# Kang-ChangWoo/audio-depth-estimation

Hardware: AMD Instinct MI355X
Metric: depth-maps/sec (train step) (higher is better)
Workload: dtype bf16; 1 GPU; unetbaseline_model unet_256 (ngf 64) train step, BatVisionV2-shaped 256x256, batch 32/GPU, Combined L1+SIlog loss, clip 1.0, AdamW; global_batch=32, image_size=256, launch=hipGraph, parallelism=dp1

## Files before the change

audio-depth-estimation_amd/csrc/epilogue.h:

```cpp
#pragma once
#include "adn_common.h"

__device__ __forceinline__ float adn_final_act(float y, int kind) {
  return kind == 1 ? 1.0f / (1.0f + __expf(-y)) : (kind == 2 ? y : fmaxf(y, 0.0f));
}

template <typename T>
__device__ __forceinline__ void epi_scalar(int epi, const AdnEpiSeg& sg, int64_t op, int nl, float v,
                                           float& s1, float& s2) {
  const int64_t idx = op * sg.channels + nl;
  if (epi == ADN_EPI_RAW) {
    reinterpret_cast<float*>(sg.out0)[idx] = v;
  } else if (epi == ADN_EPI_Z_STATS) {
    if (sg.bias) v += sg.bias[nl];
    ElemTraits<T>::store(reinterpret_cast<T*>(sg.out0) + idx, v);
    s1 += v;
    s2 += v * v;
  } else if (epi == ADN_EPI_ACT) {
    float y = v;
    if (sg.scale) y = y * sg.scale[nl];
    if (sg.shift) y += sg.shift[nl];
    if (sg.bias) y += sg.bias[nl];
    if (sg.out0) ElemTraits<T>::store(reinterpret_cast<T*>(sg.out0) + idx, y > 0.f ? y : y * sg.slope);
    if (sg.out1) ElemTraits<T>::store(reinterpret_cast<T*>(sg.out1) + idx, fmaxf(y, 0.f));
// ... 31 lines not shown
    u32x4_t c0 = p[0], c1 = p[1];
    Chunk<float>::unpack(c0, f);
    Chunk<float>::unpack(c1, f + 4);
  }
}
template <typename T>
__device__ __forceinline__ void store8(void* base, int64_t idx, const float* f) {
  if constexpr (sizeof(T) == 2) {
    *reinterpret_cast<u32x4_t*>(reinterpret_cast<uint16_t*>(base) + idx) = Chunk<uint16_t>::pack(f);
  } else {
    u32x4_t* p = reinterpret_cast<u32x4_t*>(reinterpret_cast<float*>(base) + idx);
    p[0] = Chunk<float>::pack(f);
    p[1] = Chunk<float>::pack(f + 4);
  }
}

struct EpiCols {
  float a[8], b[8];
};

template <typename T>
__device__ __forceinline__ void epi_cols_init(int epi, const AdnEpiSeg& sg, int nl, EpiCols& c) {
#pragma unroll
  for (int e = 0; e < 8; ++e) {
    c.a[e] = 1.0f;
    c.b[e] = 0.0f;
  }
  if (epi == ADN_EPI_ACT) {
#pragma unroll
    for (int e = 0; e < 8; ++e) {
      if (sg.scale) c.a[e] = sg.scale[nl + e];
      if (sg.shift) c.b[e] = sg.shift[nl + e];
      if (sg.bias) c.b[e] += sg.bias[nl + e];
    }
  } else if (epi == ADN_EPI_BWD && sg.partials) {
#pragma unroll
    for (int e = 0; e < 8; ++e) {
      c.a[e] = sg.mean[nl + e];
      c.b[e] = sg.istd[nl + e];
    }
  } else if ((epi == ADN_EPI_FINAL || epi == ADN_EPI_Z_STATS) && sg.bias) {
#pragma unroll
    for (int e = 0; e < 8; ++e) c.b[e] = sg.bias[nl + e];
  } else if (epi == ADN_EPI_ADD) {
#pragma unroll
    for (int e = 0; e < 8; ++e) {
      if (sg.scale) c.a[e] = sg.final_act ? sg.scale[0] : sg.scale[nl + e];
      if (sg.bias) c.b[e] = sg.bias[nl + e];
    }
  }
}

template <typename T>
__device__ __forceinline__ void epi_vec8(int epi, const AdnEpiSeg& sg, const EpiCols& c, int64_t op, int nl,
                                         const float* v, float* s1, float* s2) {
  const int64_t idx = op * sg.channels + nl;
  if (epi == ADN_EPI_RAW) {
    store8<float>(sg.out0, idx, v);
  } else if (epi == ADN_EPI_Z_STATS) {
    float zb[8];
#pragma unroll
    for (int e = 0; e < 8; ++e) zb[e] = v[e] + c.b[e];
    store8<T>(sg.out0, idx, zb);
#pragma unroll
    for (int e = 0; e < 8; ++e) {
      s1[e] += zb[e];
      s2[e] += zb[e] * zb[e];
    }
  } else if (epi == ADN_EPI_ACT) {
    float y[8], o[8];
#pragma unroll
    for (int e = 0; e < 8; ++e) y[e] = v[e] * c.a[e] + c.b[e];
    if (sg.out0) {
#pragma unroll
      for (int e = 0; e < 8; ++e) o[e] = y[e] > 0.f ? y[e] : y[e] * sg.slope;
      store8<T>(sg.out0, idx, o);
    }
    if (sg.out1) {
#pragma unroll
      for (int e = 0; e < 8; ++e) o[e] = fmaxf(y[e], 0.f);
      store8<T>(sg.out1, idx, o);
    }
  } else if (epi == ADN_EPI_BWD) {
    float r[8], g[8];
    load8<T>(sg.ref, idx, r);
#pragma unroll
    for (int e = 0; e < 8; ++e) g[e] = v[e] * (r[e] > 0.f ? 1.0f : sg.slope);
    if (sg.accumulate) {
      float old[8];
      load8<T>(sg.out0, idx, old);
#pragma unroll
      for (int e = 0; e < 8; ++e) g[e] += old[e];
    }
    store8<T>(sg.out0, idx, g);
    if (sg.partials) {
      float z[8];
      load8<T>(sg.z, idx, z);
#pragma unroll
      for (int e = 0; e < 8; ++e) {
        s1[e] += g[e];
        s2[e] += g[e] * ((z[e] - c.a[e]) * c.b[e]);
      }
    }
  } else if (epi == ADN_EPI_ADD) {
    float g[8];
#pragma unroll
    for (int e = 0; e < 8; ++e) g[e] = (v[e] + c.b[e]) * c.a[e];
    if (sg.ref) {
      float r[8];
      load8<T>(sg.ref, idx, r);
#pragma unroll
      for (int e = 0; e < 8; ++e) g[e] += r[e];
    }
    if (sg.accumulate) {
      float old[8];
      load8<T>(sg.out0, idx, old);
#pragma unroll
      for (int e = 0; e < 8; ++e) g[e] += old[e];
    }
    store8<T>(sg.out0, idx, g);
  } else {
    float o[8];
#pragma unroll
    for (int e = 0; e < 8; ++e) o[e] = adn_final_act(v[e] + c.b[e], sg.final_act);
    store8<float>(sg.out0, idx, o);
  }
}

__device__ __forceinline__ void epi_bwd_pre8(const AdnEpiSeg& sg, const EpiCols& c, int64_t op, int nl, const float* v,
                                             const u32x4_t& ref_raw, const u32x4_t& old_raw, const u32x4_t& z_raw,
                                             float* s1, float* s2) {
  const int64_t idx = op * sg.channels + nl;
  float r[8], g[8];
  Chunk<uint16_t>::unpack(ref_raw, r);
#pragma unroll
  for (int e = 0; e < 8; ++e) g[e] = v[e] * (r[e] > 0.f ? 1.0f : sg.slope);
  if (sg.accumulate) {
    float old[8];
    Chunk<uint16_t>::unpack(old_raw, old);
#pragma unroll
    for (int e = 0; e < 8; ++e) g[e] += old[e];
  }
  store8<uint16_t>(sg.out0, idx, g);
  if (sg.partials) {
    float z[8];
    Chunk<uint16_t>::unpack(z_raw, z);
#pragma unroll
    for (int e = 0; e < 8; ++e) {
      s1[e] += g[e];
      s2[e] += g[e] * ((z[e] - c.a[e]) * c.b[e]);
    }
  }
}
```

audio-depth-estimation_amd/csrc/igemm.hip:

```cpp
#include <stdarg.h>
#include <stdio.h>
#include <stdlib.h>

#include <mutex>

#include "epilogue.h"

namespace {

struct Tune {
  int bm = 0, bn = 0, ns = 0, noa = 0, nob = 0, skip = 0, patch = 1, tall = 1, pair = 1, tinycap = 4, bn_t2 = 0, onepx = 1, ring = 1, ring_sched = 1, ring_epi = 0, ring_geom = -1, ring_hs = 0, ring64n = 1;
};
const Tune& tune() {
  static Tune t;
  static std::once_flag once;
  std::call_once(once, [] {
    if (const char* e = getenv("ADN_IGEMM_BM")) t.bm = atoi(e);
    if (const char* e = getenv("ADN_IGEMM_BN")) t.bn = atoi(e);
    if (const char* e = getenv("ADN_IGEMM_NS")) t.ns = atoi(e);
#ifdef ADN_TIMING_KNOBS
    if (const char* e = getenv("ADN_IGEMM_NOA")) t.noa = atoi(e);
    if (const char* e = getenv("ADN_IGEMM_NOB")) t.nob = atoi(e);
    if (const char* e = getenv("ADN_IGEMM_SKIP")) t.skip = atoi(e);
#endif
    if (const char* e = getenv("ADN_IGEMM_PATCH")) t.patch = atoi(e);
    if (const char* e = getenv("ADN_IGEMM_TALL")) t.tall = atoi(e);
    if (const char* e = getenv("ADN_IGEMM_PAIR")) t.pair = atoi(e);
    if (const char* e = getenv("ADN_IGEMM_TINYCAP")) t.tinycap = atoi(e);
    if (const char* e = getenv("ADN_IGEMM_ONEPX")) t.onepx = atoi(e);
    if (const char* e = getenv("ADN_IGEMM_BN_T2")) t.bn_t2 = atoi(e);
    if (const char* e = getenv("ADN_IGEMM_RING")) t.ring = atoi(e);
    if (const char* e = getenv("ADN_IGEMM_RING_SCHED")) t.ring_sched = atoi(e);
    if (const char* e = getenv("ADN_IGEMM_RING_EPI")) t.ring_epi = atoi(e);
    if (const char* e = getenv("ADN_IGEMM_RING_GEOM")) t.ring_geom = atoi(e);
    if (const char* e = getenv("ADN_IGEMM_RING_HS")) t.ring_hs = atoi(e);
    if (const char* e = getenv("ADN_IGEMM_RING_N64")) t.ring64n = atoi(e);
  });
  return t;
}

struct KParams {
  const void* in0;
  const void* in1;
  const void* w;
  int Hs, Ws, C0, C1, N;
  int ks;
  int wstride;
  int Msmall;
  int ksteps;
  int nsplit;
  int tiles_m, tiles_n;
  int epi;
  AdnEpiSeg seg[2];
  float* slab;
  unsigned rec_a, rec_b;
  int skip;
  int onepx;
  int lgW, lgH;
};


__device__ __forceinline__ int xcd_remap(int bid, int nwg) {
  const int q = nwg >> 3, r = nwg & 7, xcd = bid & 7;
  return (xcd < r ? xcd * (q + 1) : r * (q + 1) + (xcd - r) * q) + (bid >> 3);
}

template <int N>
__device__ __forceinline__ void wait_vmcnt() {
  asm volatile("s_waitcnt vmcnt(%0) lgkmcnt(0)" ::"n"(N) : "memory");
}

template <int BM, int BN, int NWN, int NTHR>
struct TileEpi {
  static constexpr int NW = NTHR / 64;
  static constexpr int WN = BN / NWN;
  static constexpr int NT = WN / 16, MT = 4;
  static constexpr int CPR = BN / 8;
  static constexpr int RSTEP = NTHR / CPR;
  static constexpr int RPT = BM / RSTEP;
  static constexpr int LDC = BN + 4;
  static constexpr int lds_bytes = BM * LDC * 4;
};
enum class EpiPre { None, All, NoOld };
template <int RPT, EpiPre PRE>
struct EpiPreRegs {
  u32x4_t r[PRE == EpiPre::None ? 1 : RPT], o[PRE == EpiPre::All ? RPT : 1], z[PRE == EpiPre::None ? 1 : RPT];
};

template <int BM, int BN, int NWN, int NTHR, EpiPre PRE, typename RowOp>
__device__ __forceinline__ void tile_epi_prefetch(const KParams& p, int tile_n, RowOp row_op,
                                                  EpiPreRegs<TileEpi<BM, BN, NWN, NTHR>::RPT, PRE>& pre) {
  using E = TileEpi<BM, BN, NWN, NTHR>;
  if constexpr (PRE != EpiPre::None) {
    const int tid = threadIdx.x;
    const int n0 = tile_n * BN + (tid % E::CPR) * 8, rsub = tid / E::CPR;
    const bool first = n0 < p.seg[0].channels;
    const AdnEpiSeg& sq = first ? p.seg[0] : p.seg[1];
    const int nl0 = first ? n0 : n0 - p.seg[0].channels;
#pragma unroll
    for (int k = 0; k < E::RPT; ++k) {
      pre.r[k] = pre.z[k] = u32x4_t{0u, 0u, 0u, 0u};
      if constexpr (PRE == EpiPre::All) pre.o[k] = u32x4_t{0u, 0u, 0u, 0u};
      int64_t op;
      if (row_op(rsub + E::RSTEP * k, op)) {
        const int64_t idx = op * sq.channels + nl0;
        pre.r[k] = *reinterpret_cast<const u32x4_t*>(reinterpret_cast<const uint16_t*>(sq.ref) + idx);
        if constexpr (PRE == EpiPre::All) {
          if (sq.accumulate) pre.o[k] = *reinterpret_cast<const u32x4_t*>(reinterpret_cast<const uint16_t*>(sq.out0) + idx);
        }
        if (sq.partials) pre.z[k] = *reinterpret_cast<const u32x4_t*>(reinterpret_cast<const uint16_t*>(sq.z) + idx);
      }
    }
  }
}

template <typename T, int BM, int BN, int NWN, int NTHR, EpiPre PRE, typename RowOp>
__device__ __forceinline__ void tile_epi_finish(char* smem, const KParams& p, const f32x4_t (&acc)[4][BN / NWN / 16], int tile_n,
                                                int64_t prow, RowOp row_op, float* slab, bool pre_on,
                                                const EpiPreRegs<TileEpi<BM, BN, NWN, NTHR>::RPT, PRE>& pre) {
  using E = TileEpi<BM, BN, NWN, NTHR>;
  const int tid = threadIdx.x, lane = tid & 63;
  const int wave = __builtin_amdgcn_readfirstlane(tid >> 6);
  const int wm = wave / NWN, wn = wave % NWN;
  const int frow = lane & 15, fq = lane >> 4;
  __syncthreads();
  float* ct = reinterpret_cast<float*>(smem);
#pragma unroll
  for (int i = 0; i < E::MT; ++i)
#pragma unroll
    for (int j = 0; j < E::NT; ++j)
#pragma unroll
      for (int r = 0; r < 4; ++r)
        ct[(wm * 64 + i * 16 + 4 * fq + r) * E::LDC + wn * E::WN + j * 16 + frow] = acc[i][j][r];
  __syncthreads();

  const int cg = tid % E::CPR, rsub = tid / E::CPR;
  const int n0 = tile_n * BN + cg * 8;
  int epi = p.epi;
  AdnEpiSeg sg;
  int nl;
  if (slab != nullptr) {
    epi = ADN_EPI_RAW;
    sg = p.seg[0];
    sg.out0 = slab;
    sg.channels = p.N;
    sg.partials = nullptr;
    nl = n0;
  } else if (n0 < p.seg[0].channels) {
    sg = p.seg[0];
    nl = n0;
  } else {
    sg = p.seg[1];
    nl = n0 - p.seg[0].channels;
  }
  EpiCols cols;
  epi_cols_init<T>(epi, sg, nl, cols);
  float s1[8], s2[8];
#pragma unroll
  for (int e = 0; e < 8; ++e) s1[e] = s2[e] = 0.f;

#pragma unroll
  for (int k = 0; k < E::RPT; ++k) {
    const int row = rsub + E::RSTEP * k;
    int64_t op;
    if (!row_op(row, op)) continue;
    float v[8];
    const f32x4_t v0 = *reinterpret_cast<const f32x4_t*>(ct + row * E::LDC + cg * 8);
    const f32x4_t v1 = *reinterpret_cast<const f32x4_t*>(ct + row * E::LDC + cg * 8 + 4);
#pragma unroll
    for (int e = 0; e < 4; ++e) {
      v[e] = v0[e];
      v[4 + e] = v1[e];
    }
    if constexpr (PRE != EpiPre::None) {
      if (pre_on) {
        if constexpr (PRE == EpiPre::NoOld) {
          u32x4_t old = {0u, 0u, 0u, 0u};
          if (sg.accumulate) old = *reinterpret_cast<const u32x4_t*>(reinterpret_cast<const uint16_t*>(sg.out0) + op * sg.channels + nl);
          epi_bwd_pre8(sg, cols, op, nl, v, pre.r[k], old, pre.z[k], s1, s2);
        } else {
          epi_bwd_pre8(sg, cols, op, nl, v, pre.r[k], pre.o[k], pre.z[k], s1, s2);
        }
        continue;
      }
    }
    epi_vec8<T>(epi, sg, cols, op, nl, v, s1, s2);
  }

  if ((p.seg[0].partials != nullptr || p.seg[1].partials != nullptr) && (epi == ADN_EPI_Z_STATS || epi == ADN_EPI_BWD)) {
// ... 428 lines not shown
    const int soff = (t0 * Cin + (c << 5)) * 2;
    char* dst = Bl + (s & 1) * BBUF + wave * 1024;
#pragma unroll
    for (int k = 0; k < BK_; ++k) __builtin_amdgcn_raw_ptr_buffer_load_lds(rsw, (lptr_t)(dst + k * 4096), 16, bvo[k], soff, 0, 0);
  };

  f32x4_t acc[MT][NT];
#pragma unroll
  for (int i = 0; i < MT; ++i)
#pragma unroll
    for (int j = 0; j < NT; ++j) acc[i][j] = f32x4_t{0.f, 0.f, 0.f, 0.f};

  auto row_op = [&](int row, int64_t& op) -> bool {
    const int oy = oy0 + (row >> 4);
    const int ox = PAIR ? (row & 7) : ox0 + (row & 15);
    const int ib = PAIR ? tb + ((row >> 3) & 1) : tb;
    if constexpr (S2 || S1) op = ((int64_t)ib * Hs + oy) * Ws + ox;
    else op = ((int64_t)ib * Hl + 2 * oy + ph) * Wl + 2 * ox + pw;
    return true;
  };
  constexpr EpiPre EPRE = !PRE ? EpiPre::None : ((S2 || S1) ? EpiPre::NoOld : EpiPre::All);
  const bool pre_on = PRE && p.epi == ADN_EPI_BWD;
  EpiPreRegs<Cfg::Epi::RPT, EPRE> pre;
  if (pre_on) tile_epi_prefetch<BM, BN, NWN, NTHR, EPRE>(p, tile_n, row_op, pre);

#pragma unroll
  for (int ss = 0; ss < SEG_STEPS; ++ss) issue_patch(0, ss);
  issue_b(0);

  const int frow = lane & 15, fq = lane >> 4;
  const int qb0 = wm * 4 * MW + frow + (PAIR ? (frow >> 3) : 0);

  int s = 0;
  for (int sg = 0; sg < nseg; ++sg) {
    const char* Pb = Pl + (sg & 1) * PBUF;
#pragma unroll
    for (int ss = 0; ss < SEG_STEPS; ++ss, ++s) {
      wait_vmcnt<0>();
      __builtin_amdgcn_s_barrier();
      asm volatile("" ::: "memory");
      if (s + 1 < nsteps) issue_b(s + 1);
      if (sg + 1 < nseg) issue_patch(sg + 1, ss);
      const char* Bb = Bl + (s & 1) * BBUF;
#pragma unroll
      for (int e = 0; e < TPS; ++e) {
        int qoff;
        if constexpr (S2) qoff = ((e * (TH + 1)) + (ss >> 1)) * MW + (ss & 1);
        else if constexpr (S1) qoff = ss * MW + e;
        else qoff = (adn_t2_dy(ph, ss) - ymin) * MW + (adn_t2_dy(pw, e) - xmin);
        u32x4_t af[MT], bf[NT];
#pragma unroll
        for (int i = 0; i < MT; ++i) {
          const int q = qb0 + i * MW + qoff;
          af[i] = *reinterpret_cast<const u32x4_t*>(Pb + q * 64 + ((fq ^ (((q >> 2) & 1) << 1)) << 4));
        }
#pragma unroll
        for (int j = 0; j < NT; ++j) {
          const int row = wn * WN + j * 16 + frow;
          bf[j] = *reinterpret_cast<const u32x4_t*>(Bb + e * (BN * 64) + row * 64 + ((fq ^ (((row >> 2) & 1) << 1)) << 4));
        }
#pragma unroll
        for (int i = 0; i < MT; ++i)
#pragma unroll
          for (int j = 0; j < NT; ++j) mma_tile<T>(af[i], bf[j], acc[i][j]);
      }
    }
  }
  tile_epi_finish<T, BM, BN, NWN, NTHR, EPRE>(smem, p, acc, tile_n, (int64_t)phase * p.tiles_m + tile_m, row_op, nullptr, pre_on, pre);
#endif
}

#include "igemm_ring.h"

template <typename T, int GEOM>
__global__ __launch_bounds__(256) void igemm_direct_kernel(KParams p) {
  const int Hs = p.Hs, Ws = p.Ws, Hl = 2 * Hs, Wl = 2 * Ws;
  const int Cin = p.C0 + p.C1;
  const int64_t mout = (GEOM == ADN_GEMM_T2) ? (int64_t)p.Msmall * 4 : (int64_t)p.Msmall;
  const int64_t total = mout * p.N;
  const T* in0 = reinterpret_cast<const T*>(p.in0);
  const T* in1 = reinterpret_cast<const T*>(p.in1);
  const T* w = reinterpret_cast<const T*>(p.w);
  for (int64_t e = (int64_t)blockIdx.x * 256 + threadIdx.x; e < total; e += (int64_t)gridDim.x * 256) {
    const int64_t op = e / p.N;
    const int n = (int)(e - op * p.N);
    float acc = 0.f;
    auto dot = [&](int64_t pix, const T* wr) {
      for (int c = 0; c < p.C0; ++c) acc += ElemTraits<T>::load(in0 + pix * p.C0 + c) * ElemTraits<T>::load(wr + c);
      for (int c = 0; c < p.C1; ++c) acc += ElemTraits<T>::load(in1 + pix * p.C1 + c) * ElemTraits<T>::load(wr + p.C0 + c);
    };
    if constexpr (GEOM == ADN_GEMM_S2) {
      const int b = (int)(op / (Hs * Ws));
      const int rem = (int)(op - (int64_t)b * (Hs * Ws));
      const int oy = rem / Ws, ox = rem - oy * Ws;
      for (int tap = 0; tap < 16; ++tap) {
        const int iy = 2 * oy - 1 + (tap >> 2), ix = 2 * ox - 1 + (tap & 3);
        if ((unsigned)iy >= (unsigned)Hl || (unsigned)ix >= (unsigned)Wl) continue;
        const int64_t pix = ((int64_t)b * Hl + iy) * Wl + ix;
        const T* wr = w + (int64_t)n * p.wstride + tap * Cin;
        dot(pix, wr);
      }
    } else if constexpr (GEOM == ADN_GEMM_S1) {
      const int b = (int)(op / (Hs * Ws));
      const int rem = (int)(op - (int64_t)b * (Hs * Ws));
      const int oy = rem / Ws, ox = rem - oy * Ws;
      const int ks = p.ks, kpad = p.ks >> 1;
      for (int tap = 0; tap < ks * ks; ++tap) {
        const int iy = oy + tap / ks - kpad, ix = ox + tap % ks - kpad;
        if ((unsigned)iy >= (unsigned)Hs || (unsigned)ix >= (unsigned)Ws) continue;
        const int64_t pix = ((int64_t)b * Hs + iy) * Ws + ix;
        const T* wr = w + (int64_t)n * p.wstride + tap * Cin;
        dot(pix, wr);
      }
    } else {
      const int b = (int)(op / ((int64_t)Hl * Wl));
      const int rem = (int)(op - (int64_t)b * Hl * Wl);
      const int oy = rem / Wl, ox = rem - oy * Wl;
      const int ph = oy & 1, pw = ox & 1, i = oy >> 1, jx = ox >> 1;
      const int phase = ph * 2 + pw;
      for (int t = 0; t < 4; ++t) {
        const int iy = i + adn_t2_dy(ph, t >> 1), ix = jx + adn_t2_dy(pw, t & 1);
        if ((unsigned)iy >= (unsigned)Hs || (unsigned)ix >= (unsigned)Ws) continue;
        const int64_t pix = ((int64_t)b * Hs + iy) * Ws + ix;
        const T* wr = w + ((int64_t)phase * p.N + n) * p.wstride + t * Cin;
        dot(pix, wr);
      }
    }
    p.slab[e] = acc;
  }
}

template <typename T>
__global__ __launch_bounds__(256) void igemm_reduce_kernel(KParams p, int64_t mout, int rb) {
  const int64_t row0 = (int64_t)blockIdx.x * rb;
  const int64_t slab_stride = mout * p.N;
  const int n = blockIdx.y * 256 + threadIdx.x;
  if (n >= p.N) return;
  const bool in0 = n < p.seg[0].channels;
  const AdnEpiSeg& sg = in0 ? p.seg[0] : p.seg[1];
  const int nl = in0 ? n : n - p.seg[0].channels;
  float s1 = 0.f, s2 = 0.f;
  for (int r = 0; r < rb; ++r) {
    const int64_t op = row0 + r;
    if (op >= mout) break;
    const float* src = p.slab + op * p.N + n;
    float v = 0.f;
#pragma unroll 8
    for (int s = 0; s < p.nsplit; ++s) v += src[s * slab_stride];
    epi_scalar<T>(p.epi, sg, op, nl, v, s1, s2);
  }
  if (sg.partials && (p.epi == ADN_EPI_Z_STATS || p.epi == ADN_EPI_BWD)) {
    sg.partials[((int64_t)blockIdx.x * 2 + 0) * sg.channels + nl] = s1;
    sg.partials[((int64_t)blockIdx.x * 2 + 1) * sg.channels + nl] = s2;
  }
}

inline int reduce_rows(int64_t mout, int N) {
  const int64_t cb = adn_cdiv(N, 256);
  int64_t rb = mout * cb / 1024;
  if (rb > 64) rb = 64;
  if (rb < 1) rb = 1;
  return (int)rb;
}

enum class Kind { Direct, Tile, Patch, Ring };

struct Plan {
  Kind kind;
  bool tall;
  bool pair;
  bool wide;
  bool onepx;
  int wstride;
  int rb;
  int bm, bn;
  int nsplit;
  int tiles_m, tiles_n, phases;
  int ksteps;
  int64_t mout;
  int64_t partial_rows;
  int64_t slab_bytes;
};

int plan_columns(const AdnIgemmDesc* d, bool wide, int64_t msmall) {
  const Tune& tn = tune();
  if (tn.bn) return (tn.bn == 128 && d->N % 128 == 0) ? 128 : 64;
  int bn = (d->N % 128 == 0) ? 128 : 64;
  if (d->dtype != ADN_BF16) return bn;
  if (d->geom == ADN_GEMM_T2) bn = (tn.bn_t2 == 128 && d->N % 128 == 0) ? 128 : 64;
  const int64_t t128 = adn_cdiv(msmall, 128) * (d->N / 128);
  if (d->geom == ADN_GEMM_S2 && bn == 128 && t128 >= 256 && t128 < 512) bn = 64;
  if (d->geom == ADN_GEMM_S1 && d->ks == 3 && bn == 128 && wide && d->Hs % 8 == 0 && d->Ws % 16 == 0) {
    const bool tall_ok = d->Hs % 16 == 0 && tn.tall != 0 && msmall / 256 * (d->N / 64) >= 512;
    if (tall_ok || (t128 >= 256 && t128 < 512)) bn = 64;
  }
  return bn;
}

int plan_splits(const AdnIgemmDesc* d, int64_t tiles, int ksteps, int64_t mout) {
  const Tune& tn = tune();
  int ns = 1;
  if (tiles < 256) {
    ns = (int)(512 / tiles);
    const int max_by_k = ksteps / 2 > 0 ? ksteps / 2 : 1;
    if (ns > max_by_k) ns = max_by_k;
    const bool bf16 = d->dtype == ADN_BF16;
    int cap = bf16 ? 16 : 64;
    if (bf16 && tn.tinycap > 0) {
      const int64_t by_bytes = ((int64_t)tn.tinycap << 20) / (mout * d->N * 4);
      if (by_bytes > cap) cap = by_bytes > 64 ? 64 : (int)by_bytes;
    }
    if (ns > cap) ns = cap;
    if (ns < 1) ns = 1;
  }
  if (tn.ns >= 1 && ns > tn.ns) ns = tn.ns;
  return ns;
}

void plan_unsplit(Plan* pl, Kind kind, int bm, int bn, int64_t msmall, int N) {
  pl->kind = kind;
  pl->bm = bm;
  pl->bn = bn;
  pl->tiles_m = (int)(msmall / bm);
  pl->tiles_n = N / bn;
  pl->nsplit = 1;
  pl->partial_rows = (int64_t)pl->tiles_m * pl->phases;
  pl->slab_bytes = 0;
}

void make_plan(const AdnIgemmDesc* d, Plan* pl) {
  const Tune& tn = tune();
  const bool bf16 = d->dtype == ADN_BF16;
  const int esz = bf16 ? 2 : 4;
  const int bk = 128 / esz;
  const int Cin = d->C0 + d->C1;
  const int64_t msmall = (int64_t)d->B * d->Hs * d->Ws;
  pl->phases = d->geom == ADN_GEMM_T2 ? 4 : 1;
  pl->mout = msmall * pl->phases;
  const int taps = d->geom == ADN_GEMM_S2 ? 16 : (d->geom == ADN_GEMM_T2 ? 4 : d->ks * d->ks);
  pl->wstride = d->geom == ADN_GEMM_S1 ? (int)(adn_cdiv((int64_t)taps * Cin, bk) * bk) : taps * Cin;
  const int epc = 16 / esz;
  pl->wide = (d->C0 % bk == 0) && (d->C1 % bk == 0);
  const bool narrow_ok = (d->C1 == 0) && (d->C0 % epc == 0) && (d->geom == ADN_GEMM_S1 || (taps * Cin) % bk == 0);
  const bool aligned = (pl->wide || narrow_ok) && (d->N % 64 == 0) && (d->seg[0].channels % 64 == 0) &&
                       (d->seg[1].channels % 64 == 0);
  pl->tall = pl->pair = pl->onepx = false;
  pl->rb = reduce_rows(pl->mout, d->N);
  if (!aligned) {
    pl->kind = Kind::Direct;
    pl->bm = pl->bn = 0;
    pl->nsplit = 1;
    pl->tiles_m = pl->tiles_n = 0;
    pl->ksteps = 0;
    pl->partial_rows = adn_cdiv(pl->mout, pl->rb);
    pl->slab_bytes = pl->mout * d->N * 4;
    return;
  }
  const int bn0 = (d->N % 128 == 0) ? 128 : 64;
  const bool fills256 = adn_cdiv(msmall, 256) * (d->N / bn0) * pl->phases >= 256;
  int bm = (fills256 && (bn0 == 64 || taps * Cin / bk >= 32)) ? 256 : 128;
  if (tn.bm) bm = tn.bm == 256 ? 256 : 128;
  const int bn = plan_columns(d, pl->wide, msmall);
  pl->ksteps = pl->wstride / bk;
  pl->onepx = bf16 && pl->wide && d->Hs == 1 && d->Ws == 1 && d->geom != ADN_GEMM_S1 && tn.onepx != 0;
  if (pl->onepx) pl->ksteps = (d->geom == ADN_GEMM_S2 ? 4 : 1) * (Cin / bk);
  const int64_t tile_tiles = adn_cdiv(msmall, bm) * (d->N / bn) * pl->phases;
  const int ns = plan_splits(d, tile_tiles, pl->ksteps, pl->mout);
  const bool k4 = d->geom == ADN_GEMM_S2 || d->geom == ADN_GEMM_T2;

  const bool pair = bf16 && pl->wide && d->geom == ADN_GEMM_T2 && d->Hs == 8 && d->Ws == 8 && d->B % 2 == 0 &&
                    d->N % 128 == 0 && tn.pair != 0 && tn.patch != 0 &&
                    msmall / 128 * (d->N / 128) * pl->phases >= 128;
  const bool ring = bf16 && pl->wide && ns == 1 && !pair && k4 && d->Hs % 16 == 0 && d->Ws % 16 == 0 &&
                    (d->N % 128 == 0 || (d->N == 64 && tn.ring64n != 0)) && (d->geom == ADN_GEMM_S2 || Cin % 128 == 0) &&
                    tn.ring != 0 && pl->mout * d->N < (1ll << 31) && (d->epi == ADN_EPI_Z_STATS || d->epi == ADN_EPI_BWD) &&
                    (tn.ring_epi == 0 || tn.ring_epi == d->epi) && (tn.ring_geom < 0 || tn.ring_geom == d->geom) &&
                    (tn.ring_hs == 0 || tn.ring_hs == d->Hs);
  const bool patch = bf16 && pl->wide && ns == 1 && (d->geom != ADN_GEMM_S1 || d->ks == 3) && d->Hs % 8 == 0 &&
                     d->Ws % 16 == 0 && tn.patch != 0;

  if (pair) {
    plan_unsplit(pl, Kind::Patch, 128, 128, msmall, d->N);
    pl->pair = true;
  } else if (ring) {
    const int64_t t128 = msmall / 256 * (d->N / 128) * pl->phases;
    const int rbn = (d->N == 64 || tn.ring == 64 || (tn.ring != 128 && t128 < 192)) ? 64 : 128;
    plan_unsplit(pl, Kind::Ring, 256, rbn, msmall, d->N);
  } else if (patch) {
    pl->tall = bn == 64 && d->geom != ADN_GEMM_S2 && d->Hs % 16 == 0 && tn.tall != 0 &&
               msmall / 256 * (d->N / bn) * pl->phases >= 512;
    plan_unsplit(pl, Kind::Patch, pl->tall ? 256 : 128, bn, msmall, d->N);
  } else {
    pl->kind = Kind::Tile;
    pl->bm = bm;
    pl->bn = bn;
    pl->tiles_m = (int)adn_cdiv(msmall, bm);
    pl->tiles_n = d->N / bn;
    pl->nsplit = ns;
    pl->partial_rows = ns > 1 ? adn_cdiv(pl->mout, pl->rb) : (int64_t)pl->tiles_m * pl->phases;
    pl->slab_bytes = ns > 1 ? (int64_t)ns * pl->mout * d->N * 4 : 0;
  }
}

template <typename T, int BM_, int BN, int NWN, int GEOM, bool WIDE>
void launch_mfma(const KParams& kp, const Plan& pl, hipStream_t st) {
  constexpr int lds = TileCfg<BM_, BN, NWN>::lds_bytes;
  dim3 grid(pl.tiles_m * pl.tiles_n * pl.phases, 1, pl.nsplit);
  ADN_SET_LDS_ONCE(lds, &igemm_mfma_kernel<T, BM_, BN, NWN, GEOM, WIDE>);
  hipLaunchKernelGGL((igemm_mfma_kernel<T, BM_, BN, NWN, GEOM, WIDE>), grid, dim3(BM_ * NWN), lds, st, kp);
}

template <typename T, int GEOM, bool WIDE>
void dispatch_mfma2(const KParams& kp, const Plan& pl, hipStream_t st) {
  if (pl.bm == 256) {
    if (pl.bn == 128) launch_mfma<T, 256, 128, 2, GEOM, WIDE>(kp, pl, st);
    else launch_mfma<T, 256, 64, 1, GEOM, WIDE>(kp, pl, st);
  } else {
    if (pl.bn == 128) launch_mfma<T, 128, 128, 2, GEOM, WIDE>(kp, pl, st);
    else launch_mfma<T, 128, 64, 2, GEOM, WIDE>(kp, pl, st);
  }
}
template <typename T, int GEOM>
void dispatch_mfma(const KParams& kp, const Plan& pl, hipStream_t st) {
  if (pl.wide) dispatch_mfma2<T, GEOM, true>(kp, pl, st);
  else dispatch_mfma2<T, GEOM, false>(kp, pl, st);
}

template <int BN, int GEOM, bool TALL = false, bool PRE = true, bool PAIR = false>
void launch_patch1(const KParams& kp, const Plan& pl, hipStream_t st) {
  constexpr int lds = PatchCfg<BN, GEOM, TALL, PAIR>::lds_bytes;
  ADN_SET_LDS_ONCE(lds, &igemm_patch_kernel<BN, GEOM, TALL, PRE, PAIR>);
  dim3 grid(pl.tiles_m * pl.tiles_n * pl.phases, 1, 1);
  hipLaunchKernelGGL((igemm_patch_kernel<BN, GEOM, TALL, PRE, PAIR>), grid, dim3(256), lds, st, kp);
}
inline void launch_patch(const KParams& kp, const Plan& pl, int geom, hipStream_t st) {
  if (pl.pair) {
    launch_patch1<128, ADN_GEMM_T2, false, true, true>(kp, pl, st);
  } else if (geom == ADN_GEMM_S2) {
    if (pl.bn == 128 && kp.epi == ADN_EPI_BWD) launch_patch1<128, ADN_GEMM_S2>(kp, pl, st);
    else if (pl.bn == 128) launch_patch1<128, ADN_GEMM_S2, false, false>(kp, pl, st);
    else launch_patch1<64, ADN_GEMM_S2>(kp, pl, st);
  } else if (geom == ADN_GEMM_T2) {
    if (pl.bn == 128) launch_patch1<128, ADN_GEMM_T2>(kp, pl, st);
    else if (pl.tall && kp.epi == ADN_EPI_BWD) launch_patch1<64, ADN_GEMM_T2, true, true>(kp, pl, st);
    else if (pl.tall) launch_patch1<64, ADN_GEMM_T2, true, false>(kp, pl, st);
    else launch_patch1<64, ADN_GEMM_T2>(kp, pl, st);
  } else {
    if (pl.bn == 128) launch_patch1<128, ADN_GEMM_S1>(kp, pl, st);
    else if (pl.tall && kp.epi == ADN_EPI_BWD) launch_patch1<64, ADN_GEMM_S1, true, true>(kp, pl, st);
    else if (pl.tall) launch_patch1<64, ADN_GEMM_S1, true, false>(kp, pl, st);
    else launch_patch1<64, ADN_GEMM_S1>(kp, pl, st);
  }
}

inline int device_cus() {
  static int n = 0;
  static std::once_flag once;
  std::call_once(once, [] {
    int dev = 0;
    hipDeviceProp_t pr;
    if (hipGetDevice(&dev) == hipSuccess && hipGetDeviceProperties(&pr, dev) == hipSuccess) n = pr.multiProcessorCount;
    if (n <= 0) n = 256;
  });
  return n;
}

template <int GEOM, int BN, int SCHED>
void launch_ring1(const KParams& kp, const Plan& pl, hipStream_t st) {
  constexpr int lds = RingCfg<GEOM, BN>::lds_bytes;
  ADN_SET_LDS_ONCE(lds, &igemm_ring_kernel<GEOM, BN, SCHED>);
  const int ntiles = pl.tiles_m * pl.tiles_n * pl.phases;
  const int cus = device_cus();
  const int nwgs = ntiles < cus ? ntiles : cus;
  auto magic = [](int d) -> unsigned { return (unsigned)((1ull << 32) / (unsigned)d + 1ull); };
  const int tpr = kp.Ws >> 4, tpi = (kp.Hs >> 4) * tpr;
  hipLaunchKernelGGL((igemm_ring_kernel<GEOM, BN, SCHED>), dim3(nwgs), dim3(512), lds, st, kp, ntiles, nwgs,
                     pl.tiles_n == 1 ? 0u : magic(pl.tiles_n), tpi == 1 ? 0u : magic(tpi), tpr == 1 ? 0u : magic(tpr));
}
template <int GEOM, int BN>
void launch_ring2(const KParams& kp, const Plan& pl, hipStream_t st) {
  if (tune().ring_sched) launch_ring1<GEOM, BN, 1>(kp, pl, st);
  else launch_ring1<GEOM, BN, 0>(kp, pl, st);
}
inline void launch_ring(const KParams& kp, const Plan& pl, int geom, hipStream_t st) {
  if (geom == ADN_GEMM_S2) {
    if (pl.bn == 128) launch_ring2<ADN_GEMM_S2, 128>(kp, pl, st);
    else launch_ring2<ADN_GEMM_S2, 64>(kp, pl, st);
  } else {
    if (pl.bn == 128) launch_ring2<ADN_GEMM_T2, 128>(kp, pl, st);
    else launch_ring2<ADN_GEMM_T2, 64>(kp, pl, st);
  }
}

template <typename T>
int run(const AdnIgemmDesc* d, const Plan& pl, hipStream_t st) {
  KParams kp;
  kp.in0 = d->in0;
  kp.in1 = d->in1;
  kp.w = d->w;
  kp.Hs = d->Hs;
  kp.Ws = d->Ws;
  kp.C0 = d->C0;
  kp.C1 = d->C1;
  kp.N = d->N;
  kp.ks = d->geom == ADN_GEMM_S1 ? d->ks : 0;
  kp.wstride = pl.wstride;
  kp.Msmall = d->B * d->Hs * d->Ws;
  kp.ksteps = pl.ksteps;
  kp.onepx = pl.onepx ? 1 : 0;
  kp.nsplit = pl.nsplit;
  kp.tiles_m = pl.tiles_m;
  kp.tiles_n = pl.tiles_n;
  kp.epi = d->epi;
  kp.seg[0] = d->seg[0];
  kp.seg[1] = d->seg[1];
  kp.slab = reinterpret_cast<float*>(d->workspace);
  {
    auto lg2 = [](int v) { int l = 0; while ((1 << l) < v) ++l; return (1 << l) == v ? l : -1; };
    kp.lgW = lg2(d->Ws);
    kp.lgH = lg2(d->Hs);
    if (kp.lgW < 0 || kp.lgH < 0) kp.lgW = kp.lgH = -1;
  }
  kp.rec_a = tune().noa ? 0u : 0x7ffffff0u;
  kp.rec_b = tune().nob ? 0u : 0x7ffffff0u;
  kp.skip = tune().skip;
  auto reduce = [&]() {
    hipLaunchKernelGGL((igemm_reduce_kernel<T>), dim3((unsigned)adn_cdiv(pl.mout, pl.rb), (unsigned)adn_cdiv(d->N, 256)),
                       dim3(256), 0, st, kp, pl.mout, pl.rb);
  };
  switch (pl.kind) {
    case Kind::Ring:
      if constexpr (sizeof(T) == 2) launch_ring(kp, pl, d->geom, st);
      ADN_CHECK_LAUNCH();
      break;
    case Kind::Patch:
      if constexpr (sizeof(T) == 2) launch_patch(kp, pl, d->geom, st);
      ADN_CHECK_LAUNCH();
      break;
    case Kind::Tile:
      if (d->geom == ADN_GEMM_S2) dispatch_mfma<T, ADN_GEMM_S2>(kp, pl, st);
      else if (d->geom == ADN_GEMM_T2) dispatch_mfma<T, ADN_GEMM_T2>(kp, pl, st);
      else dispatch_mfma<T, ADN_GEMM_S1>(kp, pl, st);
      ADN_CHECK_LAUNCH();
      if (pl.nsplit > 1) {
        reduce();
        ADN_CHECK_LAUNCH();
      }
      break;
    case Kind::Direct: {
      const int64_t total = pl.mout * d->N;
      int64_t blocks = adn_cdiv(total, 256);
      if (blocks > 65536) blocks = 65536;
      if (d->geom == ADN_GEMM_S2)
        hipLaunchKernelGGL((igemm_direct_kernel<T, ADN_GEMM_S2>), dim3((unsigned)blocks), dim3(256), 0, st, kp);
      else if (d->geom == ADN_GEMM_T2)
        hipLaunchKernelGGL((igemm_direct_kernel<T, ADN_GEMM_T2>), dim3((unsigned)blocks), dim3(256), 0, st, kp);
      else
        hipLaunchKernelGGL((igemm_direct_kernel<T, ADN_GEMM_S1>), dim3((unsigned)blocks), dim3(256), 0, st, kp);
      ADN_CHECK_LAUNCH();
      reduce();
      ADN_CHECK_LAUNCH();
      break;
    }
  }
  return ADN_OK;
}

int validate(const AdnIgemmDesc* d) {
  ADN_CHECK_ARG(d != nullptr, "adn_igemm: null descriptor");
  ADN_CHECK_ARG(d->dtype == ADN_F32 || d->dtype == ADN_BF16, "adn_igemm: bad dtype %d", d->dtype);
  ADN_CHECK_ARG(d->geom == ADN_GEMM_S2 || d->geom == ADN_GEMM_T2 || d->geom == ADN_GEMM_S1, "adn_igemm: bad geom %d",
                d->geom);
  ADN_CHECK_ARG(d->geom != ADN_GEMM_S1 || d->ks == 1 || d->ks == 3, "adn_igemm: S1 kernel side must be 1 or 3 (got %d)",
                d->ks);
  ADN_CHECK_ARG(d->B > 0 && d->Hs > 0 && d->Ws > 0, "adn_igemm: bad shape B=%d Hs=%d Ws=%d", d->B, d->Hs, d->Ws);
  ADN_CHECK_ARG(d->C0 > 0 && d->C1 >= 0 && d->N > 0, "adn_igemm: bad channels C0=%d C1=%d N=%d", d->C0, d->C1, d->N);
  ADN_CHECK_ARG(d->in0 && d->w && (d->C1 == 0 || d->in1), "adn_igemm: null operand");
  ADN_CHECK_ARG(d->epi >= ADN_EPI_RAW && d->epi <= ADN_EPI_ADD, "adn_igemm: bad epilogue %d", d->epi);
  ADN_CHECK_ARG(d->seg[0].channels + d->seg[1].channels == d->N && d->seg[0].channels > 0 && d->seg[1].channels >= 0,
                "adn_igemm: segment channels %d+%d != N=%d", d->seg[0].channels, d->seg[1].channels, d->N);
  for (int s = 0; s < 2; ++s) {
    if (d->seg[s].channels == 0) continue;
    const AdnEpiSeg& g = d->seg[s];
    if (d->epi != ADN_EPI_ACT) ADN_CHECK_ARG(g.out0, "adn_igemm: seg %d out0 is null", s);
    if (d->epi == ADN_EPI_ACT) ADN_CHECK_ARG(g.out0 || g.out1, "adn_igemm: seg %d has no output", s);
    if (d->epi == ADN_EPI_BWD) {
      ADN_CHECK_ARG(g.ref, "adn_igemm: seg %d BWD needs ref", s);
      if (g.partials) ADN_CHECK_ARG(g.z && g.mean && g.istd, "adn_igemm: seg %d BWD stats need z/mean/istd", s);
    }
  }
  const int64_t big = (int64_t)d->B * d->Hs * d->Ws * 4;
  ADN_CHECK_ARG(big * (d->C0 + d->C1) < (1ll << 40) && big < (1ll << 31), "adn_igemm: tensor too large");
  const int64_t gpix = (int64_t)d->B * d->Hs * d->Ws * (d->geom == ADN_GEMM_S2 ? 4 : 1);
  ADN_CHECK_ARG(gpix * (d->C0 > d->C1 ? d->C0 : d->C1) * (d->dtype == ADN_BF16 ? 2 : 4) < 0x7ff00000ll,
                "adn_igemm: a gathered source exceeds 2 GiB (B=%d %dx%d C=%d/%d)", d->B, d->Hs, d->Ws, d->C0, d->C1);
  return ADN_OK;
}

}

extern "C" int64_t adn_igemm_num_partials(const AdnIgemmDesc* d) {
  if (validate(d) != ADN_OK) return -1;
  Plan pl;
  make_plan(d, &pl);
  return pl.partial_rows;
}

extern "C" int64_t adn_igemm_workspace_bytes(const AdnIgemmDesc* d) {
  if (validate(d) != ADN_OK) return -1;
  Plan pl;
  make_plan(d, &pl);
  return pl.slab_bytes;
}

extern "C" int adn_igemm_describe(const AdnIgemmDesc* d, char* buf, int len) {
  int rc = validate(d);
  if (rc != ADN_OK) return rc;
  ADN_CHECK_ARG(buf != nullptr && len > 0, "adn_igemm_describe: no buffer");
  Plan pl;
  make_plan(d, &pl);
  const char* kind = pl.kind == Kind::Direct ? "direct" : pl.kind == Kind::Ring ? "ring" : pl.kind == Kind::Tile ? "tile"
                     : pl.pair ? "patch-pair" : pl.tall ? "patch-tall" : "patch";
  snprintf(buf, (size_t)len, "%s bm=%d bn=%d nsplit=%d tiles=%dx%dx%d ksteps=%d partials=%lld ws=%lld", kind, pl.bm, pl.bn, pl.nsplit,
           pl.tiles_m, pl.tiles_n, pl.phases, pl.ksteps, (long long)pl.partial_rows, (long long)pl.slab_bytes);
  return ADN_OK;
}

extern "C" int adn_igemm(const AdnIgemmDesc* d, void* stream) {
  int rc = validate(d);
  if (rc != ADN_OK) return rc;
  Plan pl;
  make_plan(d, &pl);
  ADN_CHECK_ARG(pl.slab_bytes == 0 || (d->workspace && d->workspace_bytes >= pl.slab_bytes),
                "adn_igemm: workspace too small (%lld < %lld)", (long long)d->workspace_bytes,
                (long long)pl.slab_bytes);
  hipStream_t st = reinterpret_cast<hipStream_t>(stream);
  if (d->dtype == ADN_BF16) return run<uint16_t>(d, pl, st);
  return run<float>(d, pl, st);
}
```

Before: 13020 depth-maps/s.

## Vectorize split-K reduce kernel with 8-wide loads and epilogue-templated variants

Adds a new split-K reduction kernel where each thread handles 8 contiguous channels with 16-byte loads of the slab partials, batching several splits per iteration. Epilogue operand loads are issued before the slab summation, and per-channel statistics are staged in LDS and reduced per column. The kernel is specialized on the epilogue kind at compile time, and the old scalar kernel remains as a fallback when alignment or channel divisibility fails. The aim is fewer, wider memory transactions in the reduce pass, at the cost of LDS use and a changed summation order.

```diff
diff --git a/audio-depth-estimation_amd/csrc/epilogue.h b/audio-depth-estimation_amd/csrc/epilogue.h
--- a/audio-depth-estimation_amd/csrc/epilogue.h
+++ b/audio-depth-estimation_amd/csrc/epilogue.h
@@ -207,3 +207,144 @@
     }
   }
 }
+
+__device__ __forceinline__ float epi_unfused(float x) {
+  asm("" : "+v"(x));
+  return x;
+}
+
+template <typename T>
+struct EpiRaw8 {
+  u32x4_t c[sizeof(T) == 2 ? 1 : 2];
+};
+template <typename T>
+__device__ __forceinline__ void raw8_load(const void* base, int64_t idx, EpiRaw8<T>& r) {
+  const u32x4_t* p = reinterpret_cast<const u32x4_t*>(reinterpret_cast<const T*>(base) + idx);
+  r.c[0] = p[0];
+  if constexpr (sizeof(T) == 4) r.c[1] = p[1];
+}
+template <typename T>
+__device__ __forceinline__ void raw8_unpack(const EpiRaw8<T>& r, float* f) {
+  Chunk<T>::unpack(r.c[0], f);
+  if constexpr (sizeof(T) == 4) Chunk<T>::unpack(r.c[1], f + 4);
+}
+
+struct EpiVecs8 {
+  float a[8], b[8], c[8];
+};
+template <int EPI>
+__device__ __forceinline__ void epi_scalar8_vecs(const AdnEpiSeg& sg, int nl, EpiVecs8& k) {
+#pragma unroll
+  for (int e = 0; e < 8; ++e) {
+    if constexpr (EPI == ADN_EPI_ACT) {
+      if (sg.scale) k.a[e] = sg.scale[nl + e];
+      if (sg.shift) k.b[e] = sg.shift[nl + e];
+    } else if constexpr (EPI == ADN_EPI_BWD) {
+      if (sg.partials) {
+        k.a[e] = sg.mean[nl + e];
+        k.b[e] = sg.istd[nl + e];
+      }
+    } else if constexpr (EPI == ADN_EPI_ADD) {
+      if (sg.scale) k.a[e] = sg.final_act ? sg.scale[0] : sg.scale[nl + e];
+    }
+    if constexpr (EPI != ADN_EPI_RAW && EPI != ADN_EPI_BWD) {
+      if (sg.bias) k.c[e] = sg.bias[nl + e];
+    }
+  }
+}
+
+template <typename T>
+struct EpiOps8 {
+  EpiRaw8<T> ref, old, z;
+};
+template <typename T, int EPI>
+__device__ __forceinline__ void epi_scalar8_request(const AdnEpiSeg& sg, int64_t op, int nl, EpiOps8<T>& o) {
+  const int64_t idx = op * sg.channels + nl;
+  if constexpr (EPI == ADN_EPI_BWD) {
+    raw8_load<T>(sg.ref, idx, o.ref);
+    if (sg.accumulate) raw8_load<T>(sg.out0, idx, o.old);
+    if (sg.partials) raw8_load<T>(sg.z, idx, o.z);
+  } else if constexpr (EPI == ADN_EPI_ADD) {
+    if (sg.ref) raw8_load<T>(sg.ref, idx, o.ref);
+    if (sg.accumulate) raw8_load<T>(sg.out0, idx, o.old);
+  }
+}
+
+template <typename T, int EPI>
+__device__ __forceinline__ void epi_scalar8(const AdnEpiSeg& sg, const EpiVecs8& k, const EpiOps8<T>& o, int64_t op, int nl,
+                                            const float* v, float* t1, float* t2) {
+  const int64_t idx = op * sg.channels + nl;
+  if constexpr (EPI == ADN_EPI_RAW) {
+    store8<float>(sg.out0, idx, v);
+  } else if constexpr (EPI == ADN_EPI_Z_STATS) {
+#pragma unroll
+    for (int e = 0; e < 8; ++e) t1[e] = sg.bias ? v[e] + k.c[e] : v[e];
+    store8<T>(sg.out0, idx, t1);
+  } else if constexpr (EPI == ADN_EPI_ACT) {
+    float y[8], w[8];
+#pragma unroll
+    for (int e = 0; e < 8; ++e) {
+      y[e] = v[e];
+      if (sg.scale) y[e] = epi_unfused(y[e] * k.a[e]);
+      if (sg.shift) y[e] += k.b[e];
+      if (sg.bias) y[e] += k.c[e];
+    }
+    if (sg.out0) {
+#pragma unroll
+      for (int e = 0; e < 8; ++e) w[e] = y[e] > 0.f ? y[e] : y[e] * sg.slope;
+      store8<T>(sg.out0, idx, w);
+    }
+    if (sg.out1) {
+#pragma unroll
+      for (int e = 0; e < 8; ++e) w[e] = fmaxf(y[e], 0.f);
+      store8<T>(sg.out1, idx, w);
+    }
+  } else if constexpr (EPI == ADN_EPI_BWD) {
+    float r[8], g[8];
+    raw8_unpack<T>(o.ref, r);
+#pragma unroll
+    for (int e = 0; e < 8; ++e) g[e] = epi_unfused(v[e] * (r[e] > 0.f ? 1.0f : sg.slope));
+    if (sg.accumulate) {
+      float old[8];
+      raw8_unpack<T>(o.old, old);
+#pragma unroll
+      for (int e = 0; e < 8; ++e) g[e] += old[e];
+    }
+    store8<T>(sg.out0, idx, g);
+    if (sg.partials) {
+      float z[8];
+      raw8_unpack<T>(o.z, z);
+#pragma unroll
+      for (int e = 0; e < 8; ++e) {
+        t1[e] = g[e];
+        t2[e] = (z[e] - k.a[e]) * k.b[e];
+      }
+    }
+  } else if constexpr (EPI == ADN_EPI_ADD) {
+    float g[8];
+#pragma unroll
+    for (int e = 0; e < 8; ++e) {
+      g[e] = v[e];
+      if (sg.bias) g[e] += k.c[e];
+      if (sg.scale) g[e] = epi_unfused(g[e] * k.a[e]);
+    }
+    if (sg.ref) {
+      float r[8];
+      raw8_unpack<T>(o.ref, r);
+#pragma unroll
+      for (int e = 0; e < 8; ++e) g[e] += r[e];
+    }
+    if (sg.accumulate) {
+      float old[8];
+      raw8_unpack<T>(o.old, old);
+#pragma unroll
+      for (int e = 0; e < 8; ++e) g[e] += old[e];
+    }
+    store8<T>(sg.out0, idx, g);
+  } else {
+    float y[8];
+#pragma unroll
+    for (int e = 0; e < 8; ++e) y[e] = adn_final_act(sg.bias ? v[e] + k.c[e] : v[e], sg.final_act);
+    store8<float>(sg.out0, idx, y);
+  }
+}
diff --git a/audio-depth-estimation_amd/csrc/igemm.hip b/audio-depth-estimation_amd/csrc/igemm.hip
--- a/audio-depth-estimation_amd/csrc/igemm.hip
+++ b/audio-depth-estimation_amd/csrc/igemm.hip
@@ -1,6 +1,7 @@
 #include <stdarg.h>
 #include <stdio.h>
 #include <stdlib.h>
+#include <string.h>
 
 #include <mutex>
 
@@ -9,7 +10,7 @@
 namespace {
 
 struct Tune {
-  int bm = 0, bn = 0, ns = 0, noa = 0, nob = 0, skip = 0, patch = 1, tall = 1, pair = 1, tinycap = 4, bn_t2 = 0, onepx = 1, ring = 1, ring_sched = 1, ring_epi = 0, ring_geom = -1, ring_hs = 0, ring64n = 1;
+  int bm = 0, bn = 0, ns = 0, noa = 0, nob = 0, skip = 0, patch = 1, tall = 1, pair = 1, tinycap = 4, bn_t2 = 0, onepx = 1, ring = 1, ring_sched = 1, ring_epi = 0, ring_geom = -1, ring_hs = 0, ring64n = 1, reduce_vec = 1;
 };
 const Tune& tune() {
   static Tune t;
@@ -35,6 +36,7 @@
     if (const char* e = getenv("ADN_IGEMM_RING_GEOM")) t.ring_geom = atoi(e);
     if (const char* e = getenv("ADN_IGEMM_RING_HS")) t.ring_hs = atoi(e);
     if (const char* e = getenv("ADN_IGEMM_RING_N64")) t.ring64n = atoi(e);
+    if (const char* e = getenv("ADN_IGEMM_REDUCE")) t.reduce_vec = strcmp(e, "scalar") != 0;
   });
   return t;
 }
@@ -769,6 +771,96 @@
   if (sg.partials && (p.epi == ADN_EPI_Z_STATS || p.epi == ADN_EPI_BWD)) {
     sg.partials[((int64_t)blockIdx.x * 2 + 0) * sg.channels + nl] = s1;
     sg.partials[((int64_t)blockIdx.x * 2 + 1) * sg.channels + nl] = s2;
+  }
+}
+
+template <int G>
+__device__ __forceinline__ void slab_group_add(const float* src, int64_t slab_stride, float* v) {
+  f32x4_t x[G][2];
+#pragma unroll
+  for (int j = 0; j < G; ++j) {
+    const f32x4_t* q = reinterpret_cast<const f32x4_t*>(src + j * slab_stride);
+    x[j][0] = q[0];
+    x[j][1] = q[1];
+  }
+#pragma unroll
+  for (int j = 0; j < G; ++j) {
+#pragma unroll
+    for (int e = 0; e < 8; ++e) v[e] += x[j][e >> 2][e & 3];
+  }
+}
+
+template <typename T, int EPI>
+__global__ __launch_bounds__(256) void igemm_reduce_vec_kernel(KParams p, int64_t mout, int rb) {
+  constexpr bool STATS = EPI == ADN_EPI_Z_STATS || EPI == ADN_EPI_BWD;
+  constexpr int GMAX = (EPI == ADN_EPI_BWD && sizeof(T) == 4) ? 2
+                       : (EPI == ADN_EPI_ACT || EPI == ADN_EPI_BWD || EPI == ADN_EPI_ADD) ? 4 : 8;
+  extern __shared__ float reduce_terms[];
+  const int64_t row0 = (int64_t)blockIdx.x * rb;
+  const int64_t slab_stride = mout * p.N;
+  const int cg = threadIdx.x & 31, rstep = blockDim.x >> 5;
+  const int n = blockIdx.y * 256 + cg * 8;
+  if (n < p.N) {
+    const bool in0 = n < p.seg[0].channels;
+    const AdnEpiSeg& sg = in0 ? p.seg[0] : p.seg[1];
+    const int nl = in0 ? n : n - p.seg[0].channels;
+    EpiVecs8 k;
+    epi_scalar8_vecs<EPI>(sg, nl, k);
+    for (int r = threadIdx.x >> 5; r < rb; r += rstep) {
+      const int64_t op = row0 + r;
+      if (op >= mout) break;
+      EpiOps8<T> ops;
+      epi_scalar8_request<T, EPI>(sg, op, nl, ops);
+      const float* src = p.slab + op * p.N + n;
+      float v[8];
+#pragma unroll
+      for (int e = 0; e < 8; ++e) v[e] = 0.f;
+      int s = 0;
+      if constexpr (GMAX == 8) {
+        for (; s + 8 <= p.nsplit; s += 8) slab_group_add<8>(src + s * slab_stride, slab_stride, v);
+      }
+      if constexpr (GMAX >= 4) {
+        for (; s + 4 <= p.nsplit; s += 4) slab_group_add<4>(src + s * slab_stride, slab_stride, v);
+      }
+      for (; s + 2 <= p.nsplit; s += 2) slab_group_add<2>(src + s * slab_stride, slab_stride, v);
+      if (s < p.nsplit) slab_group_add<1>(src + s * slab_stride, slab_stride, v);
+      float t1[8], t2[8];
+      epi_scalar8<T, EPI>(sg, k, ops, op, nl, v, t1, t2);
+      if constexpr (STATS) {
+        if (sg.partials) {
+          f32x4_t* d1 = reinterpret_cast<f32x4_t*>(reduce_terms + r * 256 + cg * 8);
+          d1[0] = f32x4_t{t1[0], t1[1], t1[2], t1[3]};
+          d1[1] = f32x4_t{t1[4], t1[5], t1[6], t1[7]};
+          if constexpr (EPI == ADN_EPI_BWD) {
+            f32x4_t* d2 = reinterpret_cast<f32x4_t*>(reduce_terms + (rb + r) * 256 + cg * 8);
+            d2[0] = f32x4_t{t2[0], t2[1], t2[2], t2[3]};
+            d2[1] = f32x4_t{t2[4], t2[5], t2[6], t2[7]};
+          }
+        }
+      }
+    }
+  }
+  if constexpr (STATS) {
+    __syncthreads();
+    const int64_t left = mout - row0;
+    const int rows = left < rb ? (int)left : rb;
+    for (int c = threadIdx.x; c < 256; c += blockDim.x) {
+      const int nc = blockIdx.y * 256 + c;
+      if (nc >= p.N) break;
+      const bool in0 = nc < p.seg[0].channels;
+      const AdnEpiSeg& sg = in0 ? p.seg[0] : p.seg[1];
+      if (!sg.partials) continue;
+      const int nl = in0 ? nc : nc - p.seg[0].channels;
+      float s1 = 0.f, s2 = 0.f;
+      for (int r = 0; r < rows; ++r) {
+        const float a = reduce_terms[r * 256 + c];
+        const float b = EPI == ADN_EPI_BWD ? reduce_terms[(rb + r) * 256 + c] : a;
+        s1 += a;
+        s2 += epi_unfused(a * b);
+      }
+      sg.partials[((int64_t)blockIdx.x * 2 + 0) * sg.channels + nl] = s1;
+      sg.partials[((int64_t)blockIdx.x * 2 + 1) * sg.channels + nl] = s2;
+    }
   }
 }
 
@@ -1042,8 +1134,32 @@
   kp.rec_b = tune().nob ? 0u : 0x7ffffff0u;
   kp.skip = tune().skip;
   auto reduce = [&]() {
-    hipLaunchKernelGGL((igemm_reduce_kernel<T>), dim3((unsigned)adn_cdiv(pl.mout, pl.rb), (unsigned)adn_cdiv(d->N, 256)),
-                       dim3(256), 0, st, kp, pl.mout, pl.rb);
+    const dim3 grid((unsigned)adn_cdiv(pl.mout, pl.rb), (unsigned)adn_cdiv(d->N, 256));
+    const bool stats = d->epi == ADN_EPI_Z_STATS || d->epi == ADN_EPI_BWD;
+    const size_t lds = stats ? (size_t)pl.rb * 256 * sizeof(float) * (d->epi == ADN_EPI_BWD ? 2 : 1) : 0;
+    auto aligned16 = [](const void* q) { return (reinterpret_cast<uintptr_t>(q) & 15) == 0; };
+    bool vec = tune().reduce_vec != 0 && d->N % 8 == 0 && lds <= 65536 && aligned16(kp.slab);
+    for (int s = 0; s < 2; ++s) {
+      const AdnEpiSeg& g = d->seg[s];
+      if (g.channels == 0) continue;
+      vec = vec && g.channels % 8 == 0 && aligned16(g.out0) && aligned16(g.out1) && aligned16(g.ref) && aligned16(g.z);
+    }
+    if (!vec) {
+      hipLaunchKernelGGL((igemm_reduce_kernel<T>), grid, dim3(256), 0, st, kp, pl.mout, pl.rb);
+      return;
+    }
+    const dim3 block(pl.rb >= 8 ? 256 : (pl.rb > 2 ? 32 * pl.rb : 64));
+    switch (d->epi) {
+#define ADN_REDUCE_VEC(E) \
+  case E: hipLaunchKernelGGL((igemm_reduce_vec_kernel<T, E>), grid, block, lds, st, kp, pl.mout, pl.rb); break;
+      ADN_REDUCE_VEC(ADN_EPI_RAW)
+      ADN_REDUCE_VEC(ADN_EPI_Z_STATS)
+      ADN_REDUCE_VEC(ADN_EPI_ACT)
+      ADN_REDUCE_VEC(ADN_EPI_BWD)
+      ADN_REDUCE_VEC(ADN_EPI_FINAL)
+      ADN_REDUCE_VEC(ADN_EPI_ADD)
+#undef ADN_REDUCE_VEC
+    }
   };
   switch (pl.kind) {
     case Kind::Ring:
```

Result: faster. 13170 depth-maps/s, median of 6 (+1.2%).
